# jiaxi98/cnf_ot

Measured on AMD Instinct MI355X. Metric: MC samples/sec through flow fwd+log|detJ| at dim=2, batch=65536, higher is better.
Workload: dtype f32; 1 GPU; configs[1]: OT free dim=2, batch=65536, sample_and_log_prob (RQS fwd + log|detJ|), L=2 H=16 M=2 K=5, params N(0,0.20^2) seed 42; ONE STEP = one evaluator-shaped pass of 10000 time-slices x 65536 samples (cnf_ot/utils.py:311-340), each slice its own condition t, one cnf_sample_logprob call per rank; batch=65536, dim=2, parallelism=slice-shard x1 (contiguous blocks of the step's slices; no collective)

## Files before the change

### cnf_ot_amd/_capi.py

```python
import ctypes
import os

_HERE = os.path.dirname(os.path.abspath(__file__))
LIB_PATH = os.path.join(_HERE, "lib", "libcnf_ot_amd.so")

CNF_OK = 0
CNF_ERR_INVALID = -22
CNF_ERR_UNSUPPORTED = -95
CNF_ERR_NOMEM = -12
CNF_ERR_HIP = -5


class CnfConfig(ctypes.Structure):
  _fields_ = [
    ("dim", ctypes.c_int32), ("num_layers", ctypes.c_int32),
    ("hidden_size", ctypes.c_int32), ("mlp_num_layers", ctypes.c_int32),
    ("num_bins", ctypes.c_int32),
    ("range_min", ctypes.c_float), ("range_max", ctypes.c_float),
    ("min_bin_size", ctypes.c_float), ("min_knot_slope", ctypes.c_float),
    ("periodized", ctypes.c_int32),
  ]


class CnfFieldGrid(ctypes.Structure):
# ... 55 lines not shown
  "cnf_loss_terms_grad_multi": (ctypes.c_int, [_P, ctypes.c_int32, _P, _P, _P, _P, _P, _P, _P, _P, _P, _P, _P]),
  "cnf_input_vjp": (ctypes.c_int, [_P, ctypes.c_int, _P, _P, _I64, _P, _P, _P, _I64, _P]),
  "cnf_pass_vjp": (ctypes.c_int, [_P, ctypes.c_int, _P, _P, _I64, _P, _P, _P, _P, _P, _I64, _P]),
  "cnf_neg_logprob_vjp": (ctypes.c_int, [_P, _P, _P, _I64, ctypes.c_float, _P, _P, _P, _I64, _P]),
  "cnf_kinetic_potential_vjp": (ctypes.c_int, [_P, _P, _I64, _P, ctypes.c_int32, ctypes.c_float, ctypes.c_float, ctypes.c_int32,
                                               ctypes.c_float, ctypes.c_float, _P, _P, _P, _P, _P, _P]),
  "cnf_logprob_fd": (ctypes.c_int, [_P, _P, _P, _I64, ctypes.c_float, _P, _I64, _P]),
  "cnf_logprob_fd_vjp": (ctypes.c_int, [_P, _P, _P, _I64, ctypes.c_float, _P, _P, _P, _P, _I64, _P]),
  "cnf_score_fd_vjp": (ctypes.c_int, [_P, _P, _P, _I64, ctypes.c_float, ctypes.c_float, ctypes.c_float, ctypes.c_int32,
                                      ctypes.c_float, ctypes.c_float, _P, _P, _P, _P, _I64, _P]),
  "cnf_score_residual": (ctypes.c_int, [_P, _P, _I64, _I64, ctypes.c_int32, ctypes.c_float, ctypes.c_float,
                                        ctypes.c_int32, ctypes.c_float, ctypes.c_float, _P, _P, _P, _P]),
  "cnf_term_residual": (ctypes.c_int, [ctypes.c_int32, _P, _P, _I64, _I64, ctypes.c_int32, ctypes.c_int32, ctypes.c_float,
                                       ctypes.c_float, _P, _P, _P, _P]),
  "cnf_rkl_residual": (ctypes.c_int, [_P, _P, _I64, ctypes.c_int32, ctypes.c_float, ctypes.c_float, ctypes.c_float,
                                      ctypes.c_float, _P, _P, _P, _P]),
  "cnf_adam_step": (ctypes.c_int, [_P, _P, _P, _P, _I64, ctypes.c_float, ctypes.c_float, ctypes.c_float,
                                   ctypes.c_float, _I64, _P]),
  "cnf_step_begin": (ctypes.c_int, [_P, _P]),
  "cnf_fill_normal_dev": (ctypes.c_int, [_P, _U64, _I64, _P, _P]),
  "cnf_fill_uniform_dev": (ctypes.c_int, [_P, _U64, _I64, ctypes.c_float, _P, _P]),
  "cnf_mixture_source_dev": (ctypes.c_int, [_P, _U64, _I64, _P, _P, _P, _P]),
  "cnf_adam_step_dev": (ctypes.c_int, [_P, _P, _P, _P, _I64, ctypes.c_float, ctypes.c_float, ctypes.c_float,
                                       ctypes.c_float, _P, _P]),
  "cnf_weighted_sum": (ctypes.c_int, [_P, _P, _I64, _P, _P]),
  "cnf_hopf_cole_workspace": (ctypes.c_int, [ctypes.c_double, ctypes.c_double, ctypes.c_double, _I64, _I64,
                                              ctypes.POINTER(_I64)]),
  "cnf_hopf_cole_2d": (ctypes.c_int, [ctypes.c_int32, ctypes.c_float] + [ctypes.c_double] * 6
                       + [_P, _I64, _P, _I64, _P, _P, _P, _P, _P, _P, _P, _I64, _P]),
  "cnf_hopf_cole_path_workspace": (ctypes.c_int, [ctypes.c_double, ctypes.c_double, ctypes.c_double, _I64, _I64,
                                                   ctypes.POINTER(_I64)]),
  "cnf_hopf_cole_path_2d": (ctypes.c_int, [ctypes.c_int32, ctypes.c_float] + [ctypes.c_double] * 6
                            + [ctypes.POINTER(ctypes.c_double), _I64, _P, _I64, _P, _I64, _P, _P, _P, _P, _P, _P, _P,
                               _I64, _P]),
  "cnf_eulerian_fields": (ctypes.c_int, [_P, ctypes.POINTER(CnfFieldGrid), _P, _I64, _P, _I64, ctypes.c_float, ctypes.c_float,
                                        _P, _P, _P, _P, _P]),
  "cnf_eulerian_fields_f64": (ctypes.c_int, [_P, ctypes.POINTER(CnfFieldGrid), _P, _I64, _P, _I64, ctypes.c_double,
                                            ctypes.c_double, _P, _P, _P, _P, _P]),
  "cnf_trajectories": (ctypes.c_int, [_P, _P, _I64, ctypes.c_float, _P, _I64, ctypes.c_float, _P, _P, _P]),
  "cnf_trajectories_f64": (ctypes.c_int, [_P, _P, _I64, ctypes.c_double, _P, _I64, ctypes.c_double, _P, _P, _P]),
  "cnf_strerror": (ctypes.c_char_p, [ctypes.c_int]),
  "cnf_build_arch": (ctypes.c_char_p, []),
  "cnf_config_supported": (ctypes.c_int, [_CFG]),
}
_INTERNAL = {
  "cnf_model_set_fast_math": (ctypes.c_int, [_P, ctypes.c_int]),
  "cnf_model_set_samples_per_lane": (ctypes.c_int, [_P, ctypes.c_int]),
  "cnf_model_set_mfma": (ctypes.c_int, [_P, ctypes.c_int]),
  "cnf_model_set_pwl": (ctypes.c_int, [_P, ctypes.c_int]),
  "cnf_model_set_dpar": (ctypes.c_int, [_P, ctypes.c_int]),
  "cnf_model_set_profiling": (ctypes.c_int, [_P, ctypes.c_int]),
  "cnf_model_read_profile": (ctypes.c_int, [_P, ctypes.POINTER(ctypes.c_double), ctypes.POINTER(ctypes.c_double),
                                            ctypes.POINTER(_I64), ctypes.POINTER(_I64)]),
}
PATH_NAMES = {0: "none", 1: "mlp1", 2: "mlp2", 3: "mfma", 4: "tables", 5: "loss_mlp", 6: "loss_tables", 7: "f64", 8: "detect", 9: "dpar", 10: "fields"}

_lib = None


class CnfError(RuntimeError):
  def __init__(self, code, where):
    self.code = code
    msg = lib().cnf_strerror(code).decode() if _lib is not None else str(code)
    super().__init__(f"{where}: {msg} ({code})")


def lib():
  global _lib
  if _lib is not None:
    return _lib
  if not os.path.exists(LIB_PATH):
    raise ImportError(
      f"{LIB_PATH} is missing: the cnf_ot_amd product path is hand-written HIP "
      "for gfx950 and has no CPU fallback. Build it with "
      "`python -m cnf_ot_amd.build` (needs hipcc).")
  handle = ctypes.CDLL(LIB_PATH)
  for table in (SYMBOLS, _INTERNAL):
    for name, (res, args) in table.items():
      fn = getattr(handle, name)
      fn.restype = res
      fn.argtypes = args
  _lib = handle
  return _lib


def check(code, where):
  if code != CNF_OK:
    raise CnfError(code, where)
```

### cnf_ot_amd/csrc/cnf_flow.hip

```cpp
#include "cnf_common.h"
#include <cstdlib>
#include "cnf_pwl_build.h"

#include <math.h>
#include <new>
#include <stdlib.h>
#include <string.h>

namespace cnf {


enum CMode { C_SINGLE = 0, C_PER_SAMPLE = 1, C_TILE_UNIFORM = 2, C_GENERIC = 3 };
enum AuxMode { AUX_LOGDET = 0, AUX_LOGPROB = 1 };


template <class R> struct FlowArgsT {
  ModelArgs m;
  const R* in;
  const R* c;
  R* out;
  R* aux;
  int64_t B;
  int64_t c_block;
  int32_t c_mode, aux_mode;
// ... 1516 lines not shown
    if (ws.tables) (void)hipFree(ws.tables);
    for (float* p : ws.retired) (void)hipFree(p);
    m->pwl_ws.erase(stream);
    return CNF_OK;
  }
  if (hipMalloc((void**)&ws.tables, (size_t)cnf_model_table_bytes(m) * (size_t)n_sets + 64) != hipSuccess) {
    ws.tables = nullptr; ws.sets = 0;
    return CNF_ERR_NOMEM;
  }
  if (hipMemset(reinterpret_cast<char*>(ws.tables) + (size_t)cnf_model_table_bytes(m) * (size_t)n_sets, 0, 64) != hipSuccess) {
    (void)hipFree(ws.tables); ws.tables = nullptr; ws.sets = 0;
    return CNF_ERR_HIP;
  }
  ws.sets = n_sets; ws.epoch = 0;
  return CNF_OK;
}

extern "C" int64_t cnf_model_reserved(CnfModel* m, void* stream) {
  if (!m) return CNF_ERR_INVALID;
  float* t; int64_t sets;
  pwl_workspace(m, (hipStream_t)stream, &t, &sets);
  return sets;
}

static_assert(cnf::PWL_H == 16, "pwl_network (cnf_common.h) states the tables' network");

extern "C" int cnf_model_has_tables(const CnfModel* m) { return m && pwl_network(m->cfg) ? 1 : 0; }

extern "C" int cnf_model_term_on_tables(const CnfModel* m, int64_t slice_len, int64_t n_points, int with_grad) {
  return m && pwl_term_on_tables(m, slice_len, n_points, with_grad != 0) ? 1 : 0;
}

struct SlicePlan { int64_t tps, chunk; float* tables; };

static int slice_plan(CnfModel* m, hipStream_t stream, int64_t slice_len, int64_t n_slices, int64_t tile,
                      int sets_per_slice, SlicePlan* p) {
  const int64_t PWL_MAX_SLICES = 2048;
  p->tps = (slice_len + tile - 1) / tile;
  const int64_t total = n_slices * p->tps;
  if (total > (1 << 30)) return CNF_ERR_UNSUPPORTED;
  if (m->use_pwl == 1 && (total < 2 * (int64_t)m->num_cus || slice_len < 4 * tile)) return CNF_ERR_UNSUPPORTED;
  p->chunk = n_slices < PWL_MAX_SLICES ? n_slices : PWL_MAX_SLICES;
  int64_t sets = 0;
  pwl_workspace(m, stream, &p->tables, &sets);
  if (sets / sets_per_slice < p->chunk) p->chunk = sets / sets_per_slice;
  if (p->chunk < 1) return CNF_ERR_UNSUPPORTED;
  if (m->use_pwl == 1 && p->chunk < n_slices && p->chunk * p->tps < (int64_t)m->num_cus) return CNF_ERR_UNSUPPORTED;
  return CNF_OK;
}

static void build_tables(const CnfModel* m, hipStream_t stream, const float* c, float offset, int64_t ns,
                         float* tables) {
  const int L = m->cfg.num_layers;
  hipLaunchKernelGGL(cnf::pwl_build_kernel, dim3((unsigned)(ns * L)), dim3(512), 0, stream,
                     (const float*)(m->prep + cnf::hdr_floats(5)), m->per_layer, c, offset, L, m->scd.sp_offset, tables);
}

typedef void (*PwlKernel)(const cnf::PwlArgs);

template <bool TO_BASE, bool PRECISE, bool SEEDED>
static PwlKernel flow_pwl_kernel_of(bool full, bool l2) {
  constexpr int ALL = cnf::PWL_NPIECE, WIN = cnf::PWL_LROWS;
  if (l2) return cnf::flow_pwl_kernel<5, TO_BASE, true, PRECISE, ALL, 2, SEEDED>;
  return full ? cnf::flow_pwl_kernel<5, TO_BASE, true, PRECISE, ALL, 0, SEEDED>
              : cnf::flow_pwl_kernel<5, TO_BASE, true, PRECISE, WIN, 0, SEEDED>;
}
static PwlKernel flow_pwl_kernel_of(bool to_base, bool precise, bool seeded, bool full, bool l2) {
  if (precise) return flow_pwl_kernel_of<true, true, false>(full, l2);
  if (to_base) return flow_pwl_kernel_of<true, false, false>(full, l2);
  return seeded ? flow_pwl_kernel_of<false, false, true>(full, l2) : flow_pwl_kernel_of<false, false, false>(full, l2);
}

struct NoiseSrc { uint64_t seed; int64_t first_sample, slice_stride; };

static int run_flow_pwl(CnfModel* m, bool to_base, const float* in, const float* c, int64_t c_block,
                        float* out, float* aux, int aux_mode, int64_t B, hipStream_t stream,
                        bool detect = false, const uint32_t** gate = nullptr, uint32_t* gate_epoch = nullptr,
                        const NoiseSrc* noise = nullptr, const float* built = nullptr, bool in_shared = false) {
  if (!pwl_config_ok(m)) return CNF_ERR_UNSUPPORTED;
  const int L = m->cfg.num_layers;
  const bool precise = to_base && m->precise;
  auto lds_for = [&](int lrows) {
    return (size_t)(((cnf::hdr_floats(5) + 3) & ~3) + L * cnf::pwl_ltbl(lrows)) * sizeof(float) +
           (precise ? precise_lds_bytes(5) : 0);
  };
  const bool full = lds_for(cnf::PWL_NPIECE) <= 160 * 1024;
  size_t lds = lds_for(full ? cnf::PWL_NPIECE : cnf::PWL_LROWS);
  if (lds > 160 * 1024) return CNF_ERR_UNSUPPORTED;
  const int64_t slice_len = c_block < B ? c_block : B;
  const int64_t n_slices = (B + slice_len - 1) / slice_len;
  if (n_slices > 1 && (slice_len & 1)) return CNF_ERR_UNSUPPORTED;
  if ((reinterpret_cast<uintptr_t>(in) & 15) || (reinterpret_cast<uintptr_t>(out) & 15) ||
      (reinterpret_cast<uintptr_t>(aux) & 7))
    return CNF_ERR_UNSUPPORTED;
  const int pwl_threads = cnf::PWL_MAX_THREADS;
  const size_t pwl_min_lds = 82 * 1024;
  SlicePlan plan;
  if (slice_plan(m, stream, slice_len, n_slices, 2 * pwl_threads, 1, &plan) != CNF_OK) return CNF_ERR_UNSUPPORTED;
  const int64_t tps = plan.tps, chunk = plan.chunk;
  float* tables = plan.tables;
  if (built && (chunk < n_slices || built != tables)) return CNF_ERR_UNSUPPORTED;
  if (pwl_min_lds > lds) lds = pwl_min_lds;
  const PwlKernel kern = flow_pwl_kernel_of(to_base, precise, noise != nullptr, full, full && L == 2);
  if (!ensure_lds(kern, lds)) return CNF_ERR_UNSUPPORTED;
  uint32_t* flag = nullptr;
  uint32_t epoch = 0;
  if (detect) {
    int64_t sets = 0;
    pwl_workspace(m, stream, &tables, &sets, &flag, &epoch);
    int64_t g = (B + 4095) / 4096;
    if (g > 4 * (int64_t)m->num_cus) g = 4 * (int64_t)m->num_cus;
    hipLaunchKernelGGL(cnf::cond_uniform_kernel, dim3((unsigned)g), dim3(256), 0, stream, c, B, flag, epoch);
    *gate = flag; *gate_epoch = epoch;
  }
  m->last_path = detect ? CNF_PATH_DETECT : CNF_PATH_TABLES;
  for (int64_t s0 = 0; s0 < n_slices; s0 += chunk) {
    const int64_t ns = n_slices - s0 < chunk ? n_slices - s0 : chunk;
    const int64_t first = s0 * slice_len;
    ProfScope ps(m, stream, true, (B - first) < ns * slice_len ? (B - first) : ns * slice_len, CNF_PATH_TABLES);
    if (!built) build_tables(m, stream, c + s0, 0.0f, ns, tables);
    ps.built();
    cnf::PwlArgs a;
    a.m = model_args(m);
    a.in_shared = in_shared ? 1 : 0;
    a.in = in ? in + (in_shared ? 0 : first * 2) : nullptr; a.out = out ? out + first * 2 : nullptr; a.aux = aux ? aux + first : nullptr;
    a.seed = noise ? noise->seed : 0; a.slice_stride = noise ? noise->slice_stride : 0;
    a.first_sample = noise ? noise->first_sample + s0 * noise->slice_stride : 0;
    a.tables = tables;
    a.B = (B - first) < ns * slice_len ? (B - first) : ns * slice_len;
    a.slice_len = slice_len;
    a.n_slices = (int32_t)ns; a.tiles_per_slice = (int32_t)tps; a.aux_mode = aux_mode;
    a.gate = flag; a.gate_epoch = epoch; a.gate_want = 0;
    const int64_t tiles = ns * tps;
    const int64_t want = (int64_t)m->num_cus;
    const int64_t grid = tiles < want ? tiles : want;
    hipLaunchKernelGGL(kern, dim3((unsigned)grid), dim3(pwl_threads), lds, stream, a);
    ps.done();
  }
  return hipGetLastError() == hipSuccess ? CNF_OK : CNF_ERR_HIP;
}

int cnf_internal_flow_shared(CnfModel* m, hipStream_t stream, const float* in, const float* c, int64_t slice_len,
                             int64_t n_slices, const float* tables, float* out) {
  return run_flow_pwl(m, false, in, c, slice_len, out, nullptr, 0, n_slices * slice_len, stream, false, nullptr, nullptr,
                      nullptr, tables, true);
}

int cnf_internal_build_tables(CnfModel* m, hipStream_t stream, const float* c, int64_t n, float** tables) {
  if (!pwl_config_ok(m) || n < 1) return CNF_ERR_UNSUPPORTED;
  int64_t sets = 0;
  pwl_workspace(m, stream, tables, &sets);
  if (sets < n) return CNF_ERR_UNSUPPORTED;
  build_tables(m, stream, c, 0.0f, n, *tables);
  return hipGetLastError() == hipSuccess ? CNF_OK : CNF_ERR_HIP;
}

template <class R>
static FlowArgsT<R> flow_args(const CnfModel* m, const R* in, const R* c, int64_t c_block, R* out, R* aux, int aux_mode,
                              int64_t B, int64_t tile_samples) {
  FlowArgsT<R> a;
  a.m = model_args(m);
  a.in = in; a.c = c; a.out = out; a.aux = aux;
  a.B = B; a.c_block = c_block; a.aux_mode = aux_mode; a.div_magic = m->div_magic;
  if (c_block >= B) a.c_mode = C_SINGLE;
  else if (c_block == 1) a.c_mode = C_PER_SAMPLE;
  else if (c_block % tile_samples == 0) a.c_mode = C_TILE_UNIFORM;
  else a.c_mode = C_GENERIC;
  a.gate = nullptr; a.gate_epoch = 0; a.gate_want = 0;
  a.fd2 = 0; a.fd_h = 0; a.fd_inv_dx = 0;
  a.seed = 0; a.first_sample = 0; a.slice_stride = 0;
  return a;
}

static int run_flow(CnfModel* m, bool to_base, const float* in, const float* c, int64_t c_block,
                    float* out, float* aux, int aux_mode, int64_t B, void* stream, const NoiseSrc* noise = nullptr) {
  if (!m || (!in && !noise) || (in && noise) || !c || B < 0 || c_block < 1) return CNF_ERR_INVALID;
  if (noise && (to_base || noise->first_sample < 0 || noise->slice_stride < 0)) return CNF_ERR_INVALID;
  if (noise && c_block == 1 && B > 1 && noise->slice_stride != 1) return CNF_ERR_INVALID;
  if (!out && !aux) return CNF_ERR_INVALID;
  if (!m->params_set) return CNF_ERR_INVALID;
  if (B == 0) return CNF_OK;
  if (wait_for_params(m, (hipStream_t)stream) != CNF_OK) return CNF_ERR_HIP;
  const uint32_t* gate = nullptr;
  uint32_t gate_epoch = 0;
  if (c_block == 1 && B > 1) {
    const int r = run_flow_pwl(m, to_base, in, c, B, out, aux, aux_mode, B, (hipStream_t)stream, true, &gate, &gate_epoch, noise);
    if (r != CNF_OK && r != CNF_ERR_UNSUPPORTED) return r;
  } else {
    const int r = run_flow_pwl(m, to_base, in, c, c_block, out, aux, aux_mode, B, (hipStream_t)stream, false, nullptr, nullptr, noise);
    if (r != CNF_ERR_UNSUPPORTED) return r;
  }
  int spl = m->fast_math ? samples_per_lane(m, B) : 1;
  if (spl == 2 && (size_t)(hdr_floats(m->cfg.num_bins) + 3 * m->cfg.dim * TILE * 2) * sizeof(float) +
                      precise_lds_bytes(m->cfg.num_bins) > 160 * 1024) spl = 1;
  FlowArgs a = flow_args<float>(m, in, c, c_block, out, aux, aux_mode, B, TILE * spl);
  a.gate = gate; a.gate_epoch = gate_epoch; a.gate_want = 1;
  if (noise) { a.seed = noise->seed; a.first_sample = noise->first_sample; a.slice_stride = noise->slice_stride; }
  if (!to_base) {
    const int r = launch_flow_dpar(m, a, (hipStream_t)stream);
    if (r != CNF_ERR_UNSUPPORTED) return r;
  }
  return to_base ? launch_flow<true>(m, a, spl, (hipStream_t)stream)
                 : launch_flow<false>(m, a, spl, (hipStream_t)stream);
}

extern "C" int cnf_forward_logdet(CnfModel* m, const float* x, const float* c, int64_t c_block,
                                  float* y, float* logdet, int64_t B, void* stream) {
  return run_flow(m, false, x, c, c_block, y, logdet, AUX_LOGDET, B, stream);
}
// ... 376 lines not shown
```

### cnf_ot_amd/csrc/cnf_pwl.h

```cpp
#pragma once

#include "cnf_common.h"

namespace cnf {

constexpr int PWL_H = 16;
constexpr int PWL_P = 16;
constexpr int PWL_NBP = 320;
constexpr int PWL_NG = 2048;
constexpr int PWL_NPIECE = 289;
constexpr float PWL_GMIN = -16.0f;
constexpr float PWL_GSCALE = 64.0f;
constexpr uint32_t PWL_G_INDEX = 0x1ff, PWL_G_MANY = 0x4000, PWL_G_GENERAL = 0x8000;
constexpr int PWL_NREF = 304;
constexpr int PWL_OFF_GRID = PWL_NBP;
constexpr int PWL_OFF_REF = PWL_NBP + PWL_NG / 2;
constexpr int PWL_OFF_PIECE = PWL_NBP + PWL_NG / 2 + PWL_NREF;
static_assert(PWL_OFF_PIECE % 4 == 0, "rows are read with 16-byte LDS loads");
constexpr int PWL_ROW = 36;
constexpr int PWL_TBL = PWL_OFF_PIECE + PWL_NPIECE * PWL_ROW;
constexpr int PWL_LROWS = 112;
constexpr int PWL_LTBL = PWL_OFF_PIECE + PWL_LROWS * PWL_ROW;
constexpr int pwl_ltbl(int lrows) { return PWL_OFF_PIECE + lrows * PWL_ROW; }
constexpr int PWL_N_SLOT = PWL_NBP - 1;


constexpr double PWL_FAST_LOGIT = 4.0;
constexpr double PWL_FAST_SLOPE_LO = -3.0;
constexpr double PWL_FAST_SLOPE_HI = 40.0;
constexpr int PWL_CHUNK = 64;


__device__ __forceinline__ float fma_scalar(float a, float b, float c) {
  float r;
  asm("v_fma_f32 %0, %1, %2, %3" : "=v"(r) : "v"(a), "v"(b), "v"(c));
  return r;
}

typedef const f4 __attribute__((address_space(3))) * lds_f4_ptr;

__device__ __forceinline__ int pwl_cell(float u) {
  const int cell = (int)fmaf(u, PWL_GSCALE, -PWL_GMIN * PWL_GSCALE);
  return cell < 0 ? 0 : (cell > PWL_NG - 1 ? PWL_NG - 1 : cell);
}

template <int LROWS = PWL_LROWS>
__device__ __forceinline__ void pwl_row(const float* tbl, const float* __restrict__ gtbl, int p, float u,
                                        float (&th)[PWL_P]) {
  const float du = u - tbl[PWL_OFF_REF + p];
  if (LROWS >= PWL_NPIECE || p < LROWS) {
    const lds_f4_ptr row = (lds_f4_ptr)(uintptr_t)((uint32_t)(uintptr_t)(tbl + PWL_OFF_PIECE) + __umul24((uint32_t)p, PWL_ROW * 4));
#pragma unroll
    for (int q = 0; q < 4; ++q) {
      const f4 s = row[q], t = row[4 + q];
#pragma unroll
      for (int e = 0; e < 4; ++e) th[4 * q + e] = fma_scalar(s[e], du, t[e]);
    }
  } else {
    const f4* row = reinterpret_cast<const f4*>(gtbl + PWL_OFF_PIECE + p * PWL_ROW);
#pragma unroll
    for (int q = 0; q < 4; ++q) {
      const f4 s = row[q], t = row[4 + q];
#pragma unroll
      for (int e = 0; e < 4; ++e) th[4 * q + e] = fma_scalar(s[e], du, t[e]);
    }
  }
}

__device__ __forceinline__ int pwl_piece(const float* tbl, float u, bool& general) {
  const uint32_t g = reinterpret_cast<const uint16_t*>(tbl + PWL_OFF_GRID)[pwl_cell(u)];
  general = (g & PWL_G_GENERAL) != 0;
  int p = (int)(g & PWL_G_INDEX);
  const float us = u;
  const float b0 = tbl[p], b1 = tbl[p + 1];
  p += (b0 <= us ? 1 : 0) + (b1 <= us ? 1 : 0);
  if (g & PWL_G_MANY) while (tbl[p] <= us) ++p;
  return p;
}
__device__ __forceinline__ void pwl_piece(const float* tbl, v2f u, int& px, int& py, bool& general) {
  const uint16_t* grid = reinterpret_cast<const uint16_t*>(tbl + PWL_OFF_GRID);
  const uint32_t gx = grid[pwl_cell(u.x)], gy = grid[pwl_cell(u.y)];
  general = ((gx | gy) & PWL_G_GENERAL) != 0;
  px = (int)(gx & PWL_G_INDEX); py = (int)(gy & PWL_G_INDEX);
// ... 133 lines not shown
```

### cnf_ot_amd/csrc/cnf_pwl_build.h

```cpp
#pragma once

#include "cnf_pwl.h"

namespace cnf {

__global__ __launch_bounds__(512) void pwl_build_kernel(const float* __restrict__ weights ,
                                                        int64_t per_layer, const float* __restrict__ cvals,
                                                        float c_offset, int L, double sp_offset,
                                                        float* __restrict__ tables) {
  __shared__ double a1[PWL_H], b1v[PWL_H], W1[PWL_H * PWL_H], bb1[PWL_H], Wo[PWL_H * PWL_P], bo[PWL_P];
  __shared__ double bpu[PWL_H], sbp[PWL_H];
  __shared__ double candu[PWL_NPIECE - 1], cand[PWL_NPIECE - 1];
  __shared__ double PQ[PWL_CHUNK * PWL_H * 2];
  __shared__ double RAW[PWL_CHUNK * PWL_P * 2];
  __shared__ int bad[PWL_NPIECE];
  __shared__ double urefs[PWL_CHUNK];
  __shared__ int icnt[17], ioff[17];
  __shared__ double IPQ[17 * PWL_H * 2];
  __shared__ int biv[PWL_NPIECE];
  const int tid = threadIdx.x;
  const int slice = blockIdx.x / L, l = blockIdx.x % L;
  const float* w = weights + l * per_layer;
  const double c = (double)cvals[slice] + (double)c_offset;
  const double INF = __longlong_as_double(0x7ff0000000000000LL);
  if (tid < PWL_H) {
    const double a = (double)w[PWL_H + tid], b = (double)w[tid] * c + (double)w[2 * PWL_H + tid];
    a1[tid] = a;
    b1v[tid] = b;
    bpu[tid] = a != 0.0 ? -b / a : INF;
    bb1[tid] = (double)w[3 * PWL_H + 256 + tid];
    bo[tid] = (double)w[3 * PWL_H + 256 + PWL_H + 256 + tid];
  }
  for (int i = tid; i < 256; i += blockDim.x) {
    W1[i] = (double)w[3 * PWL_H + i];
    Wo[i] = (double)w[3 * PWL_H + 256 + PWL_H + i];
  }
  __syncthreads();
  if (tid < PWL_H) {
    const double v = bpu[tid];
    int r = 0;
    for (int j = 0; j < PWL_H; ++j) r += (bpu[j] < v || (bpu[j] == v && j < tid)) ? 1 : 0;
    sbp[r] = v;
  }
  __syncthreads();
  auto test_point = [&](double lo, double hi) -> double {
    const bool fl = lo > -INF, fh = hi < INF;
    return fl && fh ? 0.5 * (lo + hi) : (fl ? lo + 1.0 : (fh ? hi - 1.0 : 0.0));
  };
  double root = INF;
  const int iv = tid / PWL_H, kk = tid % PWL_H;
  if (tid < 17 * PWL_H) {
    const double lo = iv == 0 ? -INF : sbp[iv - 1], hi = iv == PWL_H ? INF : sbp[iv];
    if (lo < INF) {
      const double u = test_point(lo, hi);
      double P = 0.0, Q = bb1[kk];
      for (int j = 0; j < PWL_H; ++j) {
        const double on = a1[j] * u + b1v[j] > 0.0 ? W1[j * PWL_H + kk] : 0.0;
        P += on * a1[j];
        Q += on * b1v[j];
      }
      IPQ[2 * tid] = P; IPQ[2 * tid + 1] = Q;
      if (lo < hi && P != 0.0) { const double r = -Q / P; if (r > lo && r < hi) root = r; }
    }
    candu[PWL_H + tid] = root;
  }
  for (int p = tid; p < PWL_NPIECE - 1; p += blockDim.x) cand[p] = INF;
  for (int p = tid; p < PWL_NPIECE; p += blockDim.x) bad[p] = 0;
  __syncthreads();
  int rank_in = 0;
  if (tid < 17 * PWL_H) {
    int cnt = 0;
    for (int j = 0; j < PWL_H; ++j) {
      const double o = candu[PWL_H + iv * PWL_H + j];
      rank_in += (o < root || (o == root && j < kk)) ? 1 : 0;
      cnt += o < INF ? 1 : 0;
    }
    if (kk == 0) icnt[iv] = cnt;
  }
  __syncthreads();
  if (tid < 17) {
    int sum = 0;
    for (int i = 0; i < tid; ++i) sum += icnt[i];
    ioff[tid] = sum;
  }
  __syncthreads();
  if (tid < 17 * PWL_H && root < INF) {
    cand[iv + ioff[iv] + rank_in] = root;
    biv[iv + ioff[iv] + rank_in] = iv;
  }
  if (tid < PWL_H && sbp[tid] < INF) {
    cand[tid + ioff[tid] + icnt[tid]] = sbp[tid];
    biv[tid + ioff[tid] + icnt[tid]] = tid;
  }
  int n1 = 0;
  for (int j = 0; j < PWL_H; ++j) n1 += sbp[j] < INF ? 1 : 0;
  const int n = n1 + ioff[16] + icnt[16];
  __syncthreads();
  float* T = tables + (int64_t)blockIdx.x * PWL_TBL;
  for (int p = tid; p < PWL_NBP; p += blockDim.x)
    T[p] = p == PWL_N_SLOT ? __int_as_float(n) : (p < n ? (float)cand[p] : __int_as_float(0x7fc00000));
  const double LOG2E_D = 1.4426950408889634;
  for (int base = 0; base <= n; base += PWL_CHUNK) {
    const int np = n + 1 - base < PWL_CHUNK ? n + 1 - base : PWL_CHUNK;
    for (int t = tid; t < np * PWL_H; t += blockDim.x) {
      const int p = base + (t >> 4), k = t & 15;
      const double lo = p == 0 ? -INF : cand[p - 1], hi = p < n ? cand[p] : INF;
      const double u = test_point(lo, hi);
      const int ivp = p < n ? biv[p] : n1;
      const double P = IPQ[2 * (ivp * PWL_H + k)], Q = IPQ[2 * (ivp * PWL_H + k) + 1];
      const bool act = P * u + Q > 0.0;
      PQ[2 * t] = act ? P : 0.0;
      PQ[2 * t + 1] = act ? Q : 0.0;
    }
    __syncthreads();
    for (int t = tid; t < np * PWL_P; t += blockDim.x) {
      const int pl = t >> 4, m = t & 15, p = base + pl;
      double S = 0.0, Tt = bo[m];
      for (int k = 0; k < PWL_H; ++k) {
        const double wo = Wo[k * PWL_P + m];
        S += wo * PQ[2 * (pl * PWL_H + k)];
        Tt += wo * PQ[2 * (pl * PWL_H + k) + 1];
      }
      const double lo = p == 0 ? -INF : cand[p - 1], hi = p < n ? cand[p] : INF;
      const double nearest = lo > 0.0 ? lo : (hi < 0.0 ? hi : 0.0);
      const float uref = (float)(nearest < (double)PWL_GMIN ? (double)PWL_GMIN : (nearest > -(double)PWL_GMIN ? -(double)PWL_GMIN : nearest));
      Tt += S * (double)uref;
      if (m == 0) {
        T[PWL_OFF_REF + p] = uref; urefs[pl] = (double)uref;
        T[PWL_OFF_PIECE + p * PWL_ROW + 2 * PWL_P] = uref;
      }
      RAW[2 * t] = S;
      RAW[2 * t + 1] = Tt;
    }
    __syncthreads();
    for (int t = tid; t < np * PWL_P; t += blockDim.x) {
      const int pl = t >> 4, m = t & 15, p = base + pl;
      double S = RAW[2 * t], Tt = RAW[2 * t + 1];
      const double lo = p == 0 ? -INF : cand[p - 1], hi = p < n ? cand[p] : INF;
      const double uref = urefs[pl];
      const double ulo = fmax(lo, (double)PWL_GMIN - 0.01), uhi = fmin(hi, -(double)PWL_GMIN + 0.01);
      bool out_of_bounds = false;
      if (m < 2 * 5) {
        const int r0 = m < 5 ? 0 : 5;
        const double uc = ulo <= uhi ? 0.5 * (ulo + uhi) : uref;
        double Mc = -INF, Mlo = -INF, Mhi = -INF;
        for (int k = r0; k < r0 + 5; ++k) {
          const double Sk = RAW[2 * (pl * PWL_P + k)], Tk = RAW[2 * (pl * PWL_P + k) + 1];
          Mc = fmax(Mc, Tk + Sk * (uc - uref));
          Mlo = fmax(Mlo, Tk + Sk * (ulo - uref));
          Mhi = fmax(Mhi, Tk + Sk * (uhi - uref));
        }
        if (ulo <= uhi)
          out_of_bounds = fmax(fabs(Mlo - Mc), fabs(Mhi - Mc)) * LOG2E_D > PWL_FAST_LOGIT;
        S *= LOG2E_D;
        Tt = (Tt - Mc) * LOG2E_D;
      } else {
        Tt += sp_offset;
        if (ulo <= uhi) {
          const double a = Tt + S * (ulo - uref), b = Tt + S * (uhi - uref);
          out_of_bounds = fmin(a, b) < PWL_FAST_SLOPE_LO || fmax(a, b) > PWL_FAST_SLOPE_HI;
        }
        S *= LOG2E_D; Tt *= LOG2E_D;
      }
      if (out_of_bounds || !(S == S) || !(Tt == Tt)) bad[p] = 1;
      float* row = T + PWL_OFF_PIECE + p * PWL_ROW;
      row[m] = (float)S;
      row[PWL_P + m] = (float)Tt;
    }
    __syncthreads();
  }
  int* delta = reinterpret_cast<int*>(PQ);
  static_assert(sizeof(double) * PWL_CHUNK * PWL_H * 2 >= sizeof(int) * (PWL_NG + 16), "scratch for the grid scan");
  constexpr int CPT = 4;
  static_assert(PWL_NG == 512 * CPT, "one thread owns four consecutive cells (512 threads)");
  for (int g = tid; g < PWL_NG + 16; g += blockDim.x) delta[g] = 0;
  __syncthreads();
  for (int p = tid; p < n; p += blockDim.x) {
    const double gb = ceil((cand[p] + 1e-4 - (double)PWL_GMIN) * (double)PWL_GSCALE);
    const int g0 = gb < 1.0 ? 1 : (gb >= (double)PWL_NG ? PWL_NG : (int)gb);
    atomicAdd(&delta[g0], 1);
  }
  __syncthreads();
  {
    const int g0 = tid * CPT;
    int c0 = delta[g0], c1 = c0 + delta[g0 + 1], c2 = c1 + delta[g0 + 2], c3 = c2 + delta[g0 + 3];
    int run = c3;
#pragma unroll
    for (int off = 1; off < 64; off <<= 1) {
      const int v = __shfl_up(run, off, 64);
      if ((tid & 63) >= off) run += v;
    }
    int* wtot = delta + PWL_NG + 8;
    __syncthreads();
    if ((tid & 63) == 63) wtot[tid >> 6] = run;
    __syncthreads();
    int before = run - c3;
    for (int w2 = 0; w2 < (tid >> 6); ++w2) before += wtot[w2];
    const int cnt[CPT] = {before + c0, before + c1, before + c2, before + c3};
#pragma unroll
    for (int i = 0; i < CPT; ++i) {
      const int g = g0 + i;
      const int lo_ = g == 0 ? 0 : cnt[i];
      const double xr = g == PWL_NG - 1 ? INF : (double)PWL_GMIN + (double)(g + 1) / (double)PWL_GSCALE + 1e-4;
      int mark = (g == 0 || g == PWL_NG - 1) ? 1 : 0;
      for (int p = lo_; p <= n && !mark; ++p) {
        mark |= bad[p];
        if (p < n && cand[p] > xr) break;
      }
      const bool many = lo_ + 2 < n && cand[lo_ + 2] <= xr;
      reinterpret_cast<uint16_t*>(T + PWL_OFF_GRID)[g] =
          (uint16_t)((uint32_t)lo_ | (mark ? PWL_G_GENERAL : 0u) | (many ? PWL_G_MANY : 0u));
    }
  }
}


}
```

### cnf_ot_amd/flows.py

```python
import math
from collections import namedtuple
from typing import Optional, Sequence, Tuple, Union

import numpy as np
import torch

from . import _capi
from .params import FlowConfig, Params, flatten

Flow = namedtuple("Flow", [
  "log_prob", "sample", "sample_and_log_prob", "forward", "inverse",
  "forward_jac", "inverse_jac", "gauge_potential",
])

_MASK64 = (1 << 64) - 1

_WRITE_EPOCH = {}


def mark_updated(flat: torch.Tensor) -> None:
  _WRITE_EPOCH[flat.data_ptr()] = _WRITE_EPOCH.get(flat.data_ptr(), 0) + 1


def _c_config(cfg: FlowConfig) -> _capi.CnfConfig:
# ... 99 lines not shown
    self._precise = True
    self._tables_ok = bool(self.lib.cnf_model_has_tables(self._h))
    self._grad_enabled = False

  def __del__(self):
    h = getattr(self, "_h", None)
    if h:
      try:
        self.lib.cnf_model_destroy(h)
      except Exception:
        pass
      self._h = None

  def load(self, params, assume_unchanged: bool = False) -> "FlowEngine":
    flat = flatten(self.cfg, params, self.device)
    key = (flat.data_ptr(), flat._version, _WRITE_EPOCH.get(flat.data_ptr(), 0))
    if assume_unchanged and self._flat is not None and key == self._flat_key:
      return self
    with _OnDevice(self.device):
      _capi.check(self.lib.cnf_model_set_params(self._h, flat.data_ptr(), _stream_ptr(self.device)),
                  "cnf_model_set_params")
    self._flat = flat
    self._flat_key = key
    return self

  def reserve(self, n_slices: int, sets_per_slice: int = 1) -> int:
    if not self._tables_ok:
      return 0
    stream = _stream_ptr(self.device)
    have = self._reserved.get(stream, 0)
    want = min(int(n_slices), 2048) * int(sets_per_slice)
    if want <= have or torch.cuda.is_current_stream_capturing():
      return have
    want = max(16, 1 << (want - 1).bit_length())
    with _OnDevice(self.device):
      _capi.check(self.lib.cnf_model_reserve(self._h, stream, want), "cnf_model_reserve")
    self._reserved[stream] = want
    return want

  def term_on_tables(self, slice_len: int, n_points: int, with_grad: bool) -> bool:
    return bool(self.lib.cnf_model_term_on_tables(self._h, int(slice_len), int(n_points), 1 if with_grad else 0))

  def grad_ready(self, grad: torch.Tensor) -> None:
    if self._flat is None:
      raise RuntimeError("load(params) before asking for gradients")
    if not self._grad_enabled:
      with _OnDevice(self.device):
        _capi.check(self.lib.cnf_grad_enable(self._h, 0), "cnf_grad_enable")
      self._grad_enabled = True
    self._check_out(grad, (self.cfg.param_count(),), "grad")

  def last_path(self) -> str:
    return _capi.PATH_NAMES.get(self.lib.cnf_model_last_path(self._h), "?")

  def set_profiling(self, on: bool) -> None:
    _capi.check(self.lib.cnf_model_set_profiling(self._h, 1 if on else 0), "cnf_model_set_profiling")

  def read_profile(self):
    f, b = _capi.ctypes.c_double(), _capi.ctypes.c_double()
    n, smp = _capi.ctypes.c_int64(), _capi.ctypes.c_int64()
    _capi.check(self.lib.cnf_model_read_profile(self._h, _capi.ctypes.byref(f), _capi.ctypes.byref(b),
                                                _capi.ctypes.byref(n), _capi.ctypes.byref(smp)),
                "cnf_model_read_profile")
    return f.value, b.value, n.value, smp.value

  def set_fast_math(self, on: bool) -> None:
    _capi.check(self.lib.cnf_model_set_fast_math(self._h, 1 if on else 0), "cnf_model_set_fast_math")

  def set_mfma(self, mode) -> None:
    _capi.check(self.lib.cnf_model_set_mfma(self._h, int(mode)), "cnf_model_set_mfma")

  def set_pwl(self, mode: int) -> None:
    _capi.check(self.lib.cnf_model_set_pwl(self._h, int(mode)), "cnf_model_set_pwl")
    self._pwl_mode = int(mode)

  def set_dpar(self, mode: int) -> None:
    _capi.check(self.lib.cnf_model_set_dpar(self._h, int(mode)), "cnf_model_set_dpar")

  def set_precise(self, on: bool) -> None:
    _capi.check(self.lib.cnf_model_set_precise(self._h, 1 if on else 0), "cnf_model_set_precise")
    self._precise = bool(on)

  def set_samples_per_lane(self, spl: int) -> None:
    _capi.check(self.lib.cnf_model_set_samples_per_lane(self._h, int(spl)), "cnf_model_set_samples_per_lane")

  def _points(self, t, what, keep_f64=False) -> torch.Tensor:
    if torch.is_tensor(t) and t.device == self.device and t.dim() == 2 and t.shape[1] == self.cfg.dim and \
        t.is_contiguous() and (t.dtype == torch.float32 or (keep_f64 and t.dtype == torch.float64)):
      return t
    if not torch.is_tensor(t):
      t = torch.as_tensor(np.asarray(t))
    if t.dim() != 2 or t.shape[1] != self.cfg.dim:
      raise ValueError(f"{what}: expected shape [B, {self.cfg.dim}], got {tuple(t.shape)}")
    dtype = torch.float64 if (keep_f64 and t.dtype == torch.float64) else torch.float32
    return t.to(device=self.device, dtype=dtype).contiguous()

  def cond(self, cond, B: int, dtype=torch.float32) -> Tuple[torch.Tensor, int]:
    if torch.is_tensor(cond) and cond.device == self.device and cond.dtype == dtype and cond.is_contiguous():
      c = cond if cond.dim() == 1 else cond.reshape(-1)
    else:
      if not torch.is_tensor(cond):
        cond = torch.as_tensor(np.asarray(cond, dtype=np.float64))
      c = cond.to(device=self.device, dtype=dtype).reshape(-1).contiguous()
    n = c.numel()
    if n == 0:
      raise ValueError("cond is empty")
# ... 666 lines not shown
```

### include/cnf_ot_amd_debug.h

```cpp
#ifndef CNF_OT_AMD_DEBUG_H
#define CNF_OT_AMD_DEBUG_H

#include "cnf_ot_amd.h"

#ifdef __cplusplus
extern "C" {
#endif

int cnf_model_set_fast_math(CnfModel *m, int on);

int cnf_model_set_samples_per_lane(CnfModel *m, int spl);

int cnf_model_set_mfma(CnfModel *m, int mode);

int cnf_model_set_pwl(CnfModel *m, int mode);

int cnf_model_set_dpar(CnfModel *m, int mode);

int cnf_model_set_profiling(CnfModel *m, int on);
int cnf_model_read_profile(CnfModel *m, double *flow_ms, double *build_ms,
                           int64_t *launches, int64_t *samples);

#ifdef __cplusplus
}
#endif
#endif
```

Before: 89.30 billion samples/s.

## Make PWL table build persistent with smaller blocks and shuffle-based reductions

```diff
diff --git a/cnf_ot_amd/_capi.py b/cnf_ot_amd/_capi.py
--- a/cnf_ot_amd/_capi.py
+++ b/cnf_ot_amd/_capi.py
@@ -131,6 +131,7 @@
   "cnf_model_set_profiling": (ctypes.c_int, [_P, ctypes.c_int]),
   "cnf_model_read_profile": (ctypes.c_int, [_P, ctypes.POINTER(ctypes.c_double), ctypes.POINTER(ctypes.c_double),
                                             ctypes.POINTER(_I64), ctypes.POINTER(_I64)]),
+  "cnf_debug_build_tables": (ctypes.c_int, [_P, _P, _I64, _P, _P]),
 }
 PATH_NAMES = {0: "none", 1: "mlp1", 2: "mlp2", 3: "mfma", 4: "tables", 5: "loss_mlp", 6: "loss_tables", 7: "f64", 8: "detect", 9: "dpar", 10: "fields"}
 
diff --git a/cnf_ot_amd/csrc/cnf_flow.hip b/cnf_ot_amd/csrc/cnf_flow.hip
--- a/cnf_ot_amd/csrc/cnf_flow.hip
+++ b/cnf_ot_amd/csrc/cnf_flow.hip
@@ -1592,8 +1592,9 @@
 static void build_tables(const CnfModel* m, hipStream_t stream, const float* c, float offset, int64_t ns,
                          float* tables) {
   const int L = m->cfg.num_layers;
-  hipLaunchKernelGGL(cnf::pwl_build_kernel, dim3((unsigned)(ns * L)), dim3(512), 0, stream,
-                     (const float*)(m->prep + cnf::hdr_floats(5)), m->per_layer, c, offset, L, m->scd.sp_offset, tables);
+  hipLaunchKernelGGL(cnf::pwl_build_kernel, dim3((unsigned)cnf::pwl_build_grid(ns, L, m->num_cus)),
+                     dim3(cnf::PWL_BUILD_THREADS), 0, stream, (const float*)(m->prep + cnf::hdr_floats(5)), m->per_layer, c,
+                     offset, L, (int)ns, m->scd.sp_offset, tables);
 }
 
 typedef void (*PwlKernel)(const cnf::PwlArgs);
@@ -1695,6 +1696,15 @@
   return hipGetLastError() == hipSuccess ? CNF_OK : CNF_ERR_HIP;
 }
 
+extern "C" int cnf_debug_build_tables(CnfModel* m, const float* c, int64_t n, float* out, void* stream) {
+  if (!m || !c || !out) return CNF_ERR_INVALID;
+  float* tables = nullptr;
+  const int r = cnf_internal_build_tables(m, (hipStream_t)stream, c, n, &tables);
+  if (r != CNF_OK) return r;
+  return hipMemcpyAsync(out, tables, (size_t)cnf_model_table_bytes(m) * (size_t)n, hipMemcpyDeviceToDevice,
+                        (hipStream_t)stream) == hipSuccess ? CNF_OK : CNF_ERR_HIP;
+}
+
 template <class R>
 static FlowArgsT<R> flow_args(const CnfModel* m, const R* in, const R* c, int64_t c_block, R* out, R* aux, int aux_mode,
                               int64_t B, int64_t tile_samples) {
diff --git a/cnf_ot_amd/csrc/cnf_pwl.h b/cnf_ot_amd/csrc/cnf_pwl.h
--- a/cnf_ot_amd/csrc/cnf_pwl.h
+++ b/cnf_ot_amd/csrc/cnf_pwl.h
@@ -28,7 +28,6 @@
 constexpr double PWL_FAST_LOGIT = 4.0;
 constexpr double PWL_FAST_SLOPE_LO = -3.0;
 constexpr double PWL_FAST_SLOPE_HI = 40.0;
-constexpr int PWL_CHUNK = 64;
 
 
 __device__ __forceinline__ float fma_scalar(float a, float b, float c) {
diff --git a/cnf_ot_amd/csrc/cnf_pwl_build.h b/cnf_ot_amd/csrc/cnf_pwl_build.h
--- a/cnf_ot_amd/csrc/cnf_pwl_build.h
+++ b/cnf_ot_amd/csrc/cnf_pwl_build.h
@@ -4,148 +4,185 @@
 
 namespace cnf {
 
-__global__ __launch_bounds__(512) void pwl_build_kernel(const float* __restrict__ weights ,
-                                                        int64_t per_layer, const float* __restrict__ cvals,
-                                                        float c_offset, int L, double sp_offset,
-                                                        float* __restrict__ tables) {
+constexpr int PWL_BUILD_THREADS = 256;
+constexpr int PWL_BUILD_PER_CU = 4;
+
+inline int64_t pwl_build_grid(int64_t ns, int L, int num_cus) {
+  int64_t per_layer = (int64_t)num_cus * PWL_BUILD_PER_CU / L;
+  if (per_layer < 1) per_layer = 1;
+  return (per_layer < ns ? per_layer : ns) * L;
+}
+
+template <int NT>
+__device__ __forceinline__ void pwl_build_tables(const float* __restrict__ weights , int64_t per_layer,
+                                                 const float* __restrict__ cvals, float c_offset, int L, int ns,
+                                                 double sp_offset, float* __restrict__ tables) {
+  static_assert(NT % 64 == 0 && PWL_NG % NT == 0 && PWL_NG / NT >= 4 && PWL_NG / NT <= 16, "see the grid scan");
   __shared__ double a1[PWL_H], b1v[PWL_H], W1[PWL_H * PWL_H], bb1[PWL_H], Wo[PWL_H * PWL_P], bo[PWL_P];
-  __shared__ double bpu[PWL_H], sbp[PWL_H];
-  __shared__ double candu[PWL_NPIECE - 1], cand[PWL_NPIECE - 1];
-  __shared__ double PQ[PWL_CHUNK * PWL_H * 2];
-  __shared__ double RAW[PWL_CHUNK * PWL_P * 2];
+  __shared__ double sbp[PWL_H];
+  __shared__ double cand[PWL_NPIECE - 1];
   __shared__ int bad[PWL_NPIECE];
-  __shared__ double urefs[PWL_CHUNK];
-  __shared__ int icnt[17], ioff[17];
+  __shared__ int icnt[17];
   __shared__ double IPQ[17 * PWL_H * 2];
   __shared__ int biv[PWL_NPIECE];
+  __shared__ int delta[PWL_NG + 16];
+  __shared__ int wtot[NT / 64];
   const int tid = threadIdx.x;
-  const int slice = blockIdx.x / L, l = blockIdx.x % L;
+  const int l = blockIdx.x % L, stride = gridDim.x / L;
   const float* w = weights + l * per_layer;
-  const double c = (double)cvals[slice] + (double)c_offset;
   const double INF = __longlong_as_double(0x7ff0000000000000LL);
+  double a1r = 0.0, w0r = 0.0, b0r = 0.0;
   if (tid < PWL_H) {
-    const double a = (double)w[PWL_H + tid], b = (double)w[tid] * c + (double)w[2 * PWL_H + tid];
-    a1[tid] = a;
-    b1v[tid] = b;
-    bpu[tid] = a != 0.0 ? -b / a : INF;
+    a1r = (double)w[PWL_H + tid]; w0r = (double)w[tid]; b0r = (double)w[2 * PWL_H + tid];
+    a1[tid] = a1r;
     bb1[tid] = (double)w[3 * PWL_H + 256 + tid];
     bo[tid] = (double)w[3 * PWL_H + 256 + PWL_H + 256 + tid];
   }
-  for (int i = tid; i < 256; i += blockDim.x) {
+  for (int i = tid; i < 256; i += NT) {
     W1[i] = (double)w[3 * PWL_H + i];
     Wo[i] = (double)w[3 * PWL_H + 256 + PWL_H + i];
   }
-  __syncthreads();
-  if (tid < PWL_H) {
-    const double v = bpu[tid];
-    int r = 0;
-    for (int j = 0; j < PWL_H; ++j) r += (bpu[j] < v || (bpu[j] == v && j < tid)) ? 1 : 0;
-    sbp[r] = v;
-  }
-  __syncthreads();
   auto test_point = [&](double lo, double hi) -> double {
     const bool fl = lo > -INF, fh = hi < INF;
     return fl && fh ? 0.5 * (lo + hi) : (fl ? lo + 1.0 : (fh ? hi - 1.0 : 0.0));
   };
-  double root = INF;
-  const int iv = tid / PWL_H, kk = tid % PWL_H;
-  if (tid < 17 * PWL_H) {
-    const double lo = iv == 0 ? -INF : sbp[iv - 1], hi = iv == PWL_H ? INF : sbp[iv];
-    if (lo < INF) {
-      const double u = test_point(lo, hi);
-      double P = 0.0, Q = bb1[kk];
+  constexpr int NROOT = 17 * PWL_H;
+  constexpr int RT = (NROOT + NT - 1) / NT;
+  const double LOG2E_D = 1.4426950408889634;
+  int slice = blockIdx.x / L;
+  if (slice >= ns) return;
+  float cf = cvals[slice];
+  for (; slice < ns; slice += stride) {
+    const float cf_next = cvals[slice + stride < ns ? slice + stride : slice];
+    const double c = (double)cf + (double)c_offset;
+    cf = cf_next;
+    int z = 0;
+    asm volatile("" : "+s"(z));
+    if (tid < PWL_H) {
+      const double b = w0r * c + b0r;
+      const double v = a1r != 0.0 ? -b / a1r : INF;
+      b1v[tid] = b;
+      int r = 0;
+#pragma unroll 4
       for (int j = 0; j < PWL_H; ++j) {
-        const double on = a1[j] * u + b1v[j] > 0.0 ? W1[j * PWL_H + kk] : 0.0;
-        P += on * a1[j];
-        Q += on * b1v[j];
-      }
-      IPQ[2 * tid] = P; IPQ[2 * tid + 1] = Q;
-      if (lo < hi && P != 0.0) { const double r = -Q / P; if (r > lo && r < hi) root = r; }
-    }
-    candu[PWL_H + tid] = root;
-  }
-  for (int p = tid; p < PWL_NPIECE - 1; p += blockDim.x) cand[p] = INF;
-  for (int p = tid; p < PWL_NPIECE; p += blockDim.x) bad[p] = 0;
-  __syncthreads();
-  int rank_in = 0;
-  if (tid < 17 * PWL_H) {
-    int cnt = 0;
-    for (int j = 0; j < PWL_H; ++j) {
-      const double o = candu[PWL_H + iv * PWL_H + j];
-      rank_in += (o < root || (o == root && j < kk)) ? 1 : 0;
-      cnt += o < INF ? 1 : 0;
-    }
-    if (kk == 0) icnt[iv] = cnt;
-  }
-  __syncthreads();
-  if (tid < 17) {
-    int sum = 0;
-    for (int i = 0; i < tid; ++i) sum += icnt[i];
-    ioff[tid] = sum;
-  }
-  __syncthreads();
-  if (tid < 17 * PWL_H && root < INF) {
-    cand[iv + ioff[iv] + rank_in] = root;
-    biv[iv + ioff[iv] + rank_in] = iv;
-  }
-  if (tid < PWL_H && sbp[tid] < INF) {
-    cand[tid + ioff[tid] + icnt[tid]] = sbp[tid];
-    biv[tid + ioff[tid] + icnt[tid]] = tid;
-  }
-  int n1 = 0;
-  for (int j = 0; j < PWL_H; ++j) n1 += sbp[j] < INF ? 1 : 0;
-  const int n = n1 + ioff[16] + icnt[16];
-  __syncthreads();
-  float* T = tables + (int64_t)blockIdx.x * PWL_TBL;
-  for (int p = tid; p < PWL_NBP; p += blockDim.x)
-    T[p] = p == PWL_N_SLOT ? __int_as_float(n) : (p < n ? (float)cand[p] : __int_as_float(0x7fc00000));
-  const double LOG2E_D = 1.4426950408889634;
-  for (int base = 0; base <= n; base += PWL_CHUNK) {
-    const int np = n + 1 - base < PWL_CHUNK ? n + 1 - base : PWL_CHUNK;
-    for (int t = tid; t < np * PWL_H; t += blockDim.x) {
-      const int p = base + (t >> 4), k = t & 15;
+        const double o = __shfl(v, j, PWL_H);
+        r += (o < v || (o == v && j < tid)) ? 1 : 0;
+      }
+      sbp[r] = v;
+    }
+    for (int p = tid; p < PWL_NPIECE - 1; p += NT) cand[p] = INF;
+    for (int p = tid; p < PWL_NPIECE; p += NT) { bad[p] = 0; biv[p] = 0; }
+    for (int g = tid; g < PWL_NG + 16; g += NT) delta[g] = 0;
+    __syncthreads();
+    double root[RT];
+    int rank_in[RT];
+#pragma unroll
+    for (int i = 0; i < RT; ++i) {
+      const int task = tid + i * NT, iv = task / PWL_H, kk = task % PWL_H;
+      root[i] = INF; rank_in[i] = 0;
+      if (task < NROOT) {
+        const double lo = iv == 0 ? -INF : sbp[iv - 1], hi = iv == PWL_H ? INF : sbp[iv];
+        if (lo < INF) {
+          const double u = test_point(lo, hi);
+          double P = 0.0, Q = bb1[kk + z];
+#pragma unroll 4
+          for (int j = 0; j < PWL_H; ++j) {
+            const double a = a1[j + z];
+            const double on = a * u + b1v[j] > 0.0 ? W1[j * PWL_H + kk + z] : 0.0;
+            P += on * a;
+            Q += on * b1v[j];
+          }
+          IPQ[2 * task] = P; IPQ[2 * task + 1] = Q;
+          if (lo < hi && P != 0.0) { const double r = -Q / P; if (r > lo && r < hi) root[i] = r; }
+        }
+        int cnt = 0, rk = 0;
+#pragma unroll 4
+        for (int j = 0; j < PWL_H; ++j) {
+          const double o = __shfl(root[i], j, PWL_H);
+          rk += (o < root[i] || (o == root[i] && j < kk)) ? 1 : 0;
+          cnt += o < INF ? 1 : 0;
+        }
+        rank_in[i] = rk;
+        if (kk == 0) icnt[iv] = cnt;
+      }
+    }
+    __syncthreads();
+    int tot = 0, ioff[RT];
+#pragma unroll
+    for (int i = 0; i < RT; ++i) ioff[i] = 0;
+    for (int j = 0; j < 17; ++j) {
+#pragma unroll
+      for (int i = 0; i < RT; ++i) if (j == (tid + i * NT) / PWL_H) ioff[i] = tot;
+      tot += icnt[j];
+    }
+#pragma unroll
+    for (int i = 0; i < RT; ++i) {
+      const int task = tid + i * NT, iv = task / PWL_H, kk = task % PWL_H;
+      if (task < NROOT && root[i] < INF) {
+        cand[iv + ioff[i] + rank_in[i]] = root[i];
+        biv[iv + ioff[i] + rank_in[i]] = iv;
+      }
+      if (task < NROOT && kk == 0 && iv < PWL_H && sbp[iv] < INF) {
+        const int q = iv + ioff[i] + icnt[iv];
+        cand[q] = sbp[iv];
+        biv[q] = iv;
+      }
+    }
+    int n1 = 0;
+    for (int j = 0; j < PWL_H; ++j) n1 += sbp[j] < INF ? 1 : 0;
+    const int n = n1 + tot;
+    __syncthreads();
+    float* T = tables + ((int64_t)slice * L + l) * PWL_TBL;
+    static_assert(PWL_NBP % 4 == 0 && PWL_TBL % 4 == 0, "16-byte stores of the breakpoints");
+    for (int q = tid; q < PWL_NBP / 4; q += NT) {
+      f4 v;
+#pragma unroll
+      for (int e = 0; e < 4; ++e) {
+        const int p = 4 * q + e;
+        v[e] = p == PWL_N_SLOT ? __int_as_float(n) : (p < n ? (float)cand[p] : __int_as_float(0x7fc00000));
+      }
+      reinterpret_cast<f4*>(T)[q] = v;
+    }
+    for (int p = tid; p < n; p += NT) {
+      const double gb = ceil((cand[p] + 1e-4 - (double)PWL_GMIN) * (double)PWL_GSCALE);
+      const int g0 = gb < 1.0 ? 1 : (gb >= (double)PWL_NG ? PWL_NG : (int)gb);
+      atomicAdd(&delta[g0], 1);
+    }
+    for (int t = tid; t < (n + 1) * PWL_P; t += NT) {
+      const int p = t >> 4, m = t & 15;
       const double lo = p == 0 ? -INF : cand[p - 1], hi = p < n ? cand[p] : INF;
       const double u = test_point(lo, hi);
       const int ivp = p < n ? biv[p] : n1;
-      const double P = IPQ[2 * (ivp * PWL_H + k)], Q = IPQ[2 * (ivp * PWL_H + k) + 1];
+      const double P = IPQ[2 * (ivp * PWL_H + m)], Q = IPQ[2 * (ivp * PWL_H + m) + 1];
       const bool act = P * u + Q > 0.0;
-      PQ[2 * t] = act ? P : 0.0;
-      PQ[2 * t + 1] = act ? Q : 0.0;
-    }
-    __syncthreads();
-    for (int t = tid; t < np * PWL_P; t += blockDim.x) {
-      const int pl = t >> 4, m = t & 15, p = base + pl;
-      double S = 0.0, Tt = bo[m];
+      const double Pm = act ? P : 0.0, Qm = act ? Q : 0.0;
+      double S = 0.0, Tt = bo[m + z];
+#pragma unroll 4
       for (int k = 0; k < PWL_H; ++k) {
-        const double wo = Wo[k * PWL_P + m];
-        S += wo * PQ[2 * (pl * PWL_H + k)];
-        Tt += wo * PQ[2 * (pl * PWL_H + k) + 1];
-      }
-      const double lo = p == 0 ? -INF : cand[p - 1], hi = p < n ? cand[p] : INF;
+        const double wo = Wo[k * PWL_P + m + z];
+        S += wo * __shfl(Pm, k, PWL_H);
+        Tt += wo * __shfl(Qm, k, PWL_H);
+      }
       const double nearest = lo > 0.0 ? lo : (hi < 0.0 ? hi : 0.0);
-      const float uref = (float)(nearest < (double)PWL_GMIN ? (double)PWL_GMIN : (nearest > -(double)PWL_GMIN ? -(double)PWL_GMIN : nearest));
-      Tt += S * (double)uref;
+      const float uref_f = (float)(nearest < (double)PWL_GMIN ? (double)PWL_GMIN : (nearest > -(double)PWL_GMIN ? -(double)PWL_GMIN : nearest));
+      Tt += S * (double)uref_f;
       if (m == 0) {
-        T[PWL_OFF_REF + p] = uref; urefs[pl] = (double)uref;
-        T[PWL_OFF_PIECE + p * PWL_ROW + 2 * PWL_P] = uref;
-      }
-      RAW[2 * t] = S;
-      RAW[2 * t + 1] = Tt;
-    }
-    __syncthreads();
-    for (int t = tid; t < np * PWL_P; t += blockDim.x) {
-      const int pl = t >> 4, m = t & 15, p = base + pl;
-      double S = RAW[2 * t], Tt = RAW[2 * t + 1];
-      const double lo = p == 0 ? -INF : cand[p - 1], hi = p < n ? cand[p] : INF;
-      const double uref = urefs[pl];
+        T[PWL_OFF_REF + p] = uref_f;
+        T[PWL_OFF_PIECE + p * PWL_ROW + 2 * PWL_P] = uref_f;
+      }
+      const double uref = (double)uref_f;
+      const int r0 = m < 5 ? 0 : 5;
+      double Sg[5], Tg[5];
+#pragma unroll
+      for (int j = 0; j < 5; ++j) { Sg[j] = __shfl(S, r0 + j, PWL_P); Tg[j] = __shfl(Tt, r0 + j, PWL_P); }
       const double ulo = fmax(lo, (double)PWL_GMIN - 0.01), uhi = fmin(hi, -(double)PWL_GMIN + 0.01);
       bool out_of_bounds = false;
       if (m < 2 * 5) {
-        const int r0 = m < 5 ? 0 : 5;
         const double uc = ulo <= uhi ? 0.5 * (ulo + uhi) : uref;
         double Mc = -INF, Mlo = -INF, Mhi = -INF;
-        for (int k = r0; k < r0 + 5; ++k) {
-          const double Sk = RAW[2 * (pl * PWL_P + k)], Tk = RAW[2 * (pl * PWL_P + k) + 1];
+#pragma unroll
+        for (int j = 0; j < 5; ++j) {
+          const double Sk = Sg[j], Tk = Tg[j];
           Mc = fmax(Mc, Tk + Sk * (uc - uref));
           Mlo = fmax(Mlo, Tk + Sk * (ulo - uref));
           Mhi = fmax(Mhi, Tk + Sk * (uhi - uref));
@@ -168,51 +205,52 @@
       row[PWL_P + m] = (float)Tt;
     }
     __syncthreads();
+    {
+      constexpr int CPT = PWL_NG / NT;
+      const int g0 = tid * CPT;
+      int own = 0;
+#pragma unroll
+      for (int i = 0; i < CPT; ++i) own += delta[g0 + i];
+      int run = own;
+#pragma unroll
+      for (int off = 1; off < 64; off <<= 1) {
+        const int v = __shfl_up(run, off, 64);
+        if ((tid & 63) >= off) run += v;
+      }
+      if ((tid & 63) == 63) wtot[tid >> 6] = run;
+      __syncthreads();
+      int count = run - own;
+      for (int w2 = 0; w2 < (tid >> 6); ++w2) count += wtot[w2];
+      uint2* grid = reinterpret_cast<uint2*>(T + PWL_OFF_GRID) + tid * (CPT / 4);
+#pragma unroll 1
+      for (int q = 0; q < CPT / 4; ++q) {
+        uint32_t cell[4];
+#pragma unroll
+        for (int i = 0; i < 4; ++i) {
+          const int g = g0 + 4 * q + i;
+          count += delta[g];
+          const int lo_ = g == 0 ? 0 : count;
+          const double xr = g == PWL_NG - 1 ? INF : (double)PWL_GMIN + (double)(g + 1) / (double)PWL_GSCALE + 1e-4;
+          int mark = (g == 0 || g == PWL_NG - 1) ? 1 : 0;
+          for (int p = lo_; p <= n && !mark; ++p) {
+            mark |= bad[p];
+            if (p < n && cand[p] > xr) break;
+          }
+          const bool many = lo_ + 2 < n && cand[lo_ + 2] <= xr;
+          cell[i] = ((uint32_t)lo_ | (mark ? PWL_G_GENERAL : 0u) | (many ? PWL_G_MANY : 0u)) & 0xffffu;
+        }
+        grid[q] = make_uint2(cell[0] | (cell[1] << 16), cell[2] | (cell[3] << 16));
+      }
+    }
+    __syncthreads();
   }
-  int* delta = reinterpret_cast<int*>(PQ);
-  static_assert(sizeof(double) * PWL_CHUNK * PWL_H * 2 >= sizeof(int) * (PWL_NG + 16), "scratch for the grid scan");
-  constexpr int CPT = 4;
-  static_assert(PWL_NG == 512 * CPT, "one thread owns four consecutive cells (512 threads)");
-  for (int g = tid; g < PWL_NG + 16; g += blockDim.x) delta[g] = 0;
-  __syncthreads();
-  for (int p = tid; p < n; p += blockDim.x) {
-    const double gb = ceil((cand[p] + 1e-4 - (double)PWL_GMIN) * (double)PWL_GSCALE);
-    const int g0 = gb < 1.0 ? 1 : (gb >= (double)PWL_NG ? PWL_NG : (int)gb);
-    atomicAdd(&delta[g0], 1);
-  }
-  __syncthreads();
-  {
-    const int g0 = tid * CPT;
-    int c0 = delta[g0], c1 = c0 + delta[g0 + 1], c2 = c1 + delta[g0 + 2], c3 = c2 + delta[g0 + 3];
-    int run = c3;
-#pragma unroll
-    for (int off = 1; off < 64; off <<= 1) {
-      const int v = __shfl_up(run, off, 64);
-      if ((tid & 63) >= off) run += v;
-    }
-    int* wtot = delta + PWL_NG + 8;
-    __syncthreads();
-    if ((tid & 63) == 63) wtot[tid >> 6] = run;
-    __syncthreads();
-    int before = run - c3;
-    for (int w2 = 0; w2 < (tid >> 6); ++w2) before += wtot[w2];
-    const int cnt[CPT] = {before + c0, before + c1, before + c2, before + c3};
-#pragma unroll
-    for (int i = 0; i < CPT; ++i) {
-      const int g = g0 + i;
-      const int lo_ = g == 0 ? 0 : cnt[i];
-      const double xr = g == PWL_NG - 1 ? INF : (double)PWL_GMIN + (double)(g + 1) / (double)PWL_GSCALE + 1e-4;
-      int mark = (g == 0 || g == PWL_NG - 1) ? 1 : 0;
-      for (int p = lo_; p <= n && !mark; ++p) {
-        mark |= bad[p];
-        if (p < n && cand[p] > xr) break;
-      }
-      const bool many = lo_ + 2 < n && cand[lo_ + 2] <= xr;
-      reinterpret_cast<uint16_t*>(T + PWL_OFF_GRID)[g] =
-          (uint16_t)((uint32_t)lo_ | (mark ? PWL_G_GENERAL : 0u) | (many ? PWL_G_MANY : 0u));
-    }
-  }
-}
-
-
-}
+}
+
+__global__ __launch_bounds__(PWL_BUILD_THREADS) void pwl_build_kernel(const float* __restrict__ weights ,
+                                                                      int64_t per_layer, const float* __restrict__ cvals,
+                                                                      float c_offset, int L, int ns, double sp_offset,
+                                                                      float* __restrict__ tables) {
+  pwl_build_tables<PWL_BUILD_THREADS>(weights, per_layer, cvals, c_offset, L, ns, sp_offset, tables);
+}
+
+}
diff --git a/cnf_ot_amd/flows.py b/cnf_ot_amd/flows.py
--- a/cnf_ot_amd/flows.py
+++ b/cnf_ot_amd/flows.py
@@ -175,6 +175,18 @@
 
   def last_path(self) -> str:
     return _capi.PATH_NAMES.get(self.lib.cnf_model_last_path(self._h), "?")
+
+  def debug_build_tables(self, cond) -> torch.Tensor:
+    c = torch.as_tensor(cond, dtype=torch.float32, device=self.device).reshape(-1).contiguous()
+    n = c.numel()
+    if n < 1 or self.reserve(n) < n:
+      raise ValueError("debug_build_tables: 1 .. 2048 conditions on a configuration that has tables")
+    L = self.cfg.num_layers
+    out = torch.empty((n, L, self.lib.cnf_model_table_bytes(self._h) // (4 * L)), dtype=torch.float32, device=self.device)
+    with _OnDevice(self.device):
+      _capi.check(self.lib.cnf_debug_build_tables(self._h, c.data_ptr(), n, out.data_ptr(), _stream_ptr(self.device)),
+                  "cnf_debug_build_tables")
+    return out
 
   def set_profiling(self, on: bool) -> None:
     _capi.check(self.lib.cnf_model_set_profiling(self._h, 1 if on else 0), "cnf_model_set_profiling")
diff --git a/include/cnf_ot_amd_debug.h b/include/cnf_ot_amd_debug.h
--- a/include/cnf_ot_amd_debug.h
+++ b/include/cnf_ot_amd_debug.h
@@ -21,6 +21,8 @@
 int cnf_model_read_profile(CnfModel *m, double *flow_ms, double *build_ms,
                            int64_t *launches, int64_t *samples);
 
+int cnf_debug_build_tables(CnfModel *m, const float *c, int64_t n, float *out, void *stream);
+
 #ifdef __cplusplus
 }
 #endif
```

Measured after the change: 89.68 billion samples/s, median of 6. Within noise of the previous version (+0.4%).
